# williamyang1991/VToonify

Measured on NVIDIA H100. Metric: frames/sec at 576x1024, higher is better.
Workload: dtype bf16x3 (fp32 operands split into bf16 hi+lo, 3 tensor-core products, fp32 accumulate)

## Files before the change

vtoonify_b200/_lib.py:

```python
import ctypes
import os
from ctypes import POINTER, Structure, c_char_p, c_float, c_int, c_int32, c_int64, c_void_p

_HERE = os.path.dirname(os.path.abspath(__file__))
LIB_PATH = os.path.join(_HERE, "lib", "libvtoonify_b200.so")
ABI_VERSION = 6
VT_MAX_TAPS = 36
ACT_NONE, ACT_LRELU, ACT_RELU_TANH = 0, 1, 2


class VtError(RuntimeError):
    pass


class ConvDesc(Structure):
    _fields_ = [
        ("struct_size", c_int32), ("n_src", c_int32),
        ("src", c_void_p * 2), ("src_c", c_int32 * 2), ("src_cstride", c_int32 * 2),
        ("B", c_int32), ("H", c_int32), ("W", c_int32), ("Ho", c_int32), ("Wo", c_int32),
        ("stride", c_int32), ("taps", c_int32),
        ("tap_dy", c_int32 * VT_MAX_TAPS), ("tap_dx", c_int32 * VT_MAX_TAPS), ("tap_w", c_int32 * VT_MAX_TAPS),
        ("tap_phase", c_int32 * VT_MAX_TAPS), ("n_phase", c_int32), ("out_cpitch", c_int32), ("phase_off", c_int64 * 4),
        ("weight", c_void_p), ("wB", c_int32), ("w_taps", c_int32), ("w_cstride", c_int32), ("Cout", c_int32),
        ("out", c_void_p), ("out_sb", c_int64), ("out_sy", c_int64), ("out_sx", c_int64),
# ... 83 lines not shown
    if _lib is not None:
        return _lib
    if not os.path.exists(LIB_PATH):
        raise VtError(
            f"{LIB_PATH} is missing: build it with `python -c 'import __graft_entry__ as g; g.build()'` "
            "(or vtoonify_b200/csrc/build.sh). vtoonify_b200 has no CPU / PyTorch fallback.")
    lib = ctypes.CDLL(LIB_PATH)
    for name, (res, args) in SYMBOLS.items():
        fn = getattr(lib, name)
        fn.restype = res
        fn.argtypes = args
    if lib.vt_abi_version() != ABI_VERSION:
        raise VtError(f"ABI mismatch: library reports {lib.vt_abi_version()}, binding expects {ABI_VERSION}")
    for env, key in (("VT_TC_MODE", b"tc_mode"), ("VT_TC_MT", b"tc_mt"), ("VT_TC_TGROUP", b"tc_tgroup"),
                     ("VT_TC_STAGE_POLICY", b"tc_stage_policy"), ("VT_TC_HALO_PCT", b"tc_halo_pct"), ("VT_TC_M_MAJOR", b"tc_m_major"),
                     ("VT_INSTNORM_CHUNKS", b"instnorm_chunks")):
        if os.environ.get(env) is not None and os.environ.get(env) != "":
            lib.vt_set_option(key, int(os.environ[env]))
    _lib = lib
    return lib


def check(status):
    if status != 0:
        raise VtError(load().vt_last_error().decode("utf-8", "replace"))


def launch_count():
    return int(load().vt_launch_count())
```

vtoonify_b200/csrc/conv_tc.cu:

```cuda
#include "tc_common.cuh"
#include <cuda_bf16.h>
#include <mutex>

using namespace vt_tc;

int vt_validate_conv_desc(const vt_conv_desc* d, const char* who);
extern int g_upfirdn_tiled;
extern int g_smalln_is;
extern int g_fir4;
extern int g_instnorm_chunks;

namespace {

constexpr int TILE_W = 8, TILE_H = 16, TILE_M = 128;
constexpr int KCH = 32;
constexpr int MAX_SMEM = 227 * 1024;
constexpr int MAX_BLOCK_N = 128;
constexpr int MAX_ACC_COLS = 128;
constexpr int STATS_WARPS = 8;

struct TcArgs {
  CUtensorMap in_map[2][4];
  CUtensorMap w_map;
  int n_src, kchunks[2], coff[2];
// ... 17 lines not shown
  int64_t out_sb, out_sy, out_sx, phase_off[4];
  int64_t pix_sb, pix_sy, pix_sx, phase_pix[4];
  int act, round_tf32;
  float slope, gain, alpha, beta;
  const float* rgb_w; const float* rgb_bias; const float* rgb_skip; const float* rgb_skip_kernel; float* rgb_out;
  const float* slope_vec;
  const float* src_scale[2];
  const float* src_affine[2];
  int src_cn[2];
  int64_t sc_sb, sc_sy, sc_sx;
  int in_w, in_h;
  int mma_n;
  int m_major;
  float* stats_ws;
  float acc_scale;
};

constexpr int TC_THREADS = 384;
constexpr int XFORM_WARPS = 3;
constexpr int CONSUMERS = 2;
constexpr int RELEASE_ARRIVALS = CONSUMERS * 4;

enum TcOp : int {
  OP_TF32 = 0,
  OP_BF16 = 1,
  OP_F16 = 2,
  OP_BF16_NSTACK = 3,
};

template <int NW, bool F16>
__device__ __forceinline__ void wgmma_split(float* acc, uint64_t a, uint64_t b, uint32_t accumulate) {
  if constexpr (NW == 32) {
    if constexpr (F16) wgmma_f16_n32(acc, a, b, accumulate); else wgmma_bf16_n32(acc, a, b, accumulate);
  } else if constexpr (NW == 64) {
    if constexpr (F16) wgmma_f16_n64(acc, a, b, accumulate); else wgmma_bf16_n64(acc, a, b, accumulate);
  } else {
// ... 12 lines not shown
      wgmma_tf32_n64(acc, adesc + 4, bdesc + 4, 1); wgmma_tf32_n64(acc, adesc + 6, bdesc + 6, 1);
    } else {
      wgmma_tf32_n128(acc, adesc, bdesc, first ^ 1u); wgmma_tf32_n128(acc, adesc + 2, bdesc + 2, 1);
      wgmma_tf32_n128(acc, adesc + 4, bdesc + 4, 1); wgmma_tf32_n128(acc, adesc + 6, bdesc + 6, 1);
    }
  } else {
    constexpr bool nstack = OP == OP_BF16_NSTACK;
    constexpr int ao[6] = {0, 2, 4, 6, 0, 2};
    constexpr int bo[6] = {0, 2, 0, 2, 4, 6};
#pragma unroll
    for (int i = 0; i < (nstack ? 4 : 6); ++i)
      wgmma_split<NW, OP == OP_F16>(acc, adesc + (uint64_t)ao[i], bdesc + (uint64_t)(nstack ? ao[i] : bo[i]), i == 0 ? (first ^ 1u) : 1u);
  }
}

template <int NW, int MT, int OP>
__global__ void __launch_bounds__(TC_THREADS, 1)
conv_tc_kernel(const __grid_constant__ TcArgs p) {
  static_assert(MT * NW <= MAX_ACC_COLS && (MT == 1 || MT == 2 || MT == 4), "accumulators of one work item exceed the register plan");
  static_assert(OP != OP_BF16_NSTACK || NW == 64, "the N-stacked form is the Cout == 32 layer at MMA N = 64");
  constexpr bool SPLIT = OP != OP_TF32;
  extern __shared__ uint8_t smem_raw[];
  const uint32_t smem_base = (smem_u32(smem_raw) + 1023u) & ~1023u;
  const uint32_t a_base = smem_base;
  const uint32_t b_base = a_base + (uint32_t)p.a_stages * p.a_stage_bytes;
  const uint32_t bar_base = b_base + (uint32_t)p.b_stages * p.b_stage_bytes;
  auto a_full = [&](int i) { return bar_base + 8u * i; };
  auto a_empty = [&](int i) { return bar_base + 64u + 8u * i; };
  auto b_full = [&](int i) { return bar_base + 128u + 8u * i; };
  auto b_empty = [&](int i) { return bar_base + 192u + 8u * i; };
  auto a_ready = [&](int i) { return bar_base + 256u + 8u * i; };

  const int warp = threadIdx.x >> 5, lane = threadIdx.x & 31;
  const int wg = threadIdx.x >> 7;

  if (warp == 0 && lane == 0) {
    for (int s = 0; s < p.n_src; ++s)
      for (int v = 0; v < 4; ++v) tma_prefetch_desc(&p.in_map[s][v]);
    tma_prefetch_desc(&p.w_map);
  }
  if (warp == 1 && lane == 0) {
    for (int i = 0; i < p.a_stages; ++i) { mbar_init(a_full(i), 1); mbar_init(a_empty(i), RELEASE_ARRIVALS); mbar_init(a_ready(i), XFORM_WARPS); }
    for (int i = 0; i < p.b_stages; ++i) { mbar_init(b_full(i), 1); mbar_init(b_empty(i), RELEASE_ARRIVALS); }
    fence_barrier_init();
    fence_proxy_async_smem();
  }
  __syncthreads();

  const int m_tiles = p.B * p.tiles_y * p.tiles_x;
  const int tiles_per_img = p.tiles_y * p.tiles_x;
  constexpr int item_w = TILE_W * MT;

  if (wg == 0) {
    if (warp == 0) {
      int a_st = 0, b_st = 0;
      uint32_t a_par = 0, b_par = 0;
      for (int tile = blockIdx.x; tile < p.total_tiles; tile += gridDim.x) {
        const int n_tile = p.m_major ? tile % p.n_tiles : tile / m_tiles, m = p.m_major ? tile / p.n_tiles : tile % m_tiles;
// ... 107 lines not shown
#pragma unroll
                for (int m4 = 0; m4 < 4; ++m4) {
                  asm volatile("st.shared.v4.b32 [%0], {%1, %2, %3, %4};" ::"r"(row + ((m4 ^ ph) << 4)), "r"(hi[4 * m4]), "r"(hi[4 * m4 + 1]), "r"(hi[4 * m4 + 2]), "r"(hi[4 * m4 + 3]) : "memory");
                  asm volatile("st.shared.v4.b32 [%0], {%1, %2, %3, %4};" ::"r"(row + (((m4 + 4) ^ ph) << 4)), "r"(lo[4 * m4]), "r"(lo[4 * m4 + 1]), "r"(lo[4 * m4 + 2]), "r"(lo[4 * m4 + 3]) : "memory");
                }
              }
              fence_proxy_async_smem();
              __syncwarp();
              if (lane == 0) mbar_arrive(a_ready(a_st));
              if (++a_st == p.a_stages) { a_st = 0; a_par ^= 1; }
            }
          }
        }
      }
    }
  } else {
    const int c = wg - 1;
    const int tw_ = (threadIdx.x & 127) >> 5;
    const bool leader = lane == 0;
    const int qd = lane & 3;
    float acc[MT][NW / 2];
#pragma unroll
    for (int g = 0; g < MT; ++g)
#pragma unroll
      for (int i = 0; i < NW / 2; ++i) acc[g][i] = 0.f;
    const float nw = (p.noise && p.noise_w) ? *p.noise_w : 0.f;
    int a_st = 0, b_st = 0;
    uint32_t a_par = 0, b_par = 0;
    const uint32_t tile_bytes_n = (uint32_t)p.mma_n * 128u;
    for (int tile = blockIdx.x; tile < p.total_tiles; tile += gridDim.x) {
      const int n_tile = p.m_major ? tile % p.n_tiles : tile / m_tiles, m = p.m_major ? tile / p.n_tiles : tile % m_tiles;
      const int b = m / tiles_per_img, rem = m % tiles_per_img;
      const int oy0 = (rem / p.tiles_x) * TILE_H, ox0 = (rem % p.tiles_x) * item_w;
      const int n0 = n_tile * p.block_n;
      uint32_t first = 1;
      int rel_a = -1, rel_b = -1;
      for (int s = 0; s < p.n_src; ++s) {
        for (int kc = 0; kc < p.kchunks[s]; ++kc) {
          if (p.halo) mbar_wait(SPLIT ? a_ready(a_st) : a_full(a_st), a_par);
          int gj = 0;
          for (int j = 0; j < p.n_steps; ++j) {
            if (!p.halo) mbar_wait(SPLIT ? a_ready(a_st) : a_full(a_st), a_par);
            if (gj == 0) mbar_wait(b_full(b_st), b_par);
            uint32_t a_addr = a_base + a_st * p.a_stage_bytes;
            uint32_t sbo = 1024;
            if (p.halo) {
              a_addr += (uint32_t)p.step_aoff[j];
              sbo = (uint32_t)p.step_sbo[j];
            }
            a_addr += 8u * (uint32_t)c * sbo;
            const uint64_t bdesc = make_smem_desc_sw128(b_base + b_st * p.b_stage_bytes + (uint32_t)gj * tile_bytes_n, 1024);
            const bool last_of_group = (gj == p.tgroup - 1);
            wgmma_fence();
#pragma unroll
            for (int g = 0; g < MT; ++g) {
              const uint64_t adesc = make_smem_desc_sw128(a_addr + (uint32_t)(g * TILE_W * 128), sbo);
              mma_step<NW, OP>(acc[g], adesc, bdesc, first);
            }
            wgmma_commit();
            wgmma_wait<1>();
            if (leader) {
              if (rel_a >= 0) mbar_arrive(a_empty(rel_a));
              if (rel_b >= 0) mbar_arrive(b_empty(rel_b));
            }
            rel_a = (!p.halo || j == p.n_steps - 1) ? a_st : -1;
            rel_b = last_of_group ? b_st : -1;
            first = 0;
            if (last_of_group) { gj = 0; if (++b_st == p.b_stages) { b_st = 0; b_par ^= 1; } } else { ++gj; }
            if (!p.halo || j == p.n_steps - 1) { if (++a_st == p.a_stages) { a_st = 0; a_par ^= 1; } }
          }
        }
      }
      wgmma_wait<0>();
#pragma unroll
      for (int g = 0; g < MT; ++g) wgmma_pin<NW / 2>(acc[g]);
      if (leader) {
        if (rel_a >= 0) mbar_arrive(a_empty(rel_a));
        if (rel_b >= 0) mbar_arrive(b_empty(rel_b));
      }

      const int r0 = 64 * c + 16 * tw_ + (lane >> 2);
      const int ty = r0 / TILE_W, tx = r0 % TILE_W;
      const int ph0 = n0 / p.Cout, nb0 = n0 - ph0 * p.Cout;
      const int nchunks = p.block_n / 32;
#pragma unroll
      for (int g = 0; g < MT; ++g) {
        int oy[2], ox[2];
        bool in_img[2];
        int64_t off0[2], pix0[2];
        float rgb[2][3] = {{0.f, 0.f, 0.f}, {0.f, 0.f, 0.f}};
#pragma unroll
        for (int h = 0; h < 2; ++h) {
          oy[h] = oy0 + ty + h; ox[h] = ox0 + g * TILE_W + tx;
          in_img[h] = oy[h] < p.Ho && ox[h] < p.Wo;
          off0[h] = (int64_t)b * p.out_sb + (int64_t)oy[h] * p.out_sy + (int64_t)ox[h] * p.out_sx;
          pix0[h] = (int64_t)b * p.pix_sb + (int64_t)oy[h] * p.pix_sy + (int64_t)ox[h] * p.pix_sx;
        }
        int ph = ph0, nb = nb0 - 32;
#pragma unroll
        for (int j = 0; j < NW / 32; ++j) {
          if (j >= nchunks) break;
          nb += 32;
          if (nb >= p.Cout) { nb -= p.Cout; ++ph; }
          float nz[2];
#pragma unroll
          for (int h = 0; h < 2; ++h) nz[h] = (p.noise && in_img[h]) ? nw * __ldg(p.noise + p.phase_pix[ph] + pix0[h]) : 0.f;
          float v[2][4][2];
#pragma unroll
          for (int k = 0; k < 4; ++k)
#pragma unroll
            for (int h = 0; h < 2; ++h)
#pragma unroll
              for (int e = 0; e < 2; ++e) {
                const int i = 16 * j + 4 * k + 2 * h + e;
                float x = acc[g][i];
                if constexpr (OP == OP_BF16_NSTACK) x += acc[g][(i + 16) % (NW / 2)];
                v[h][k][e] = x * p.acc_scale;
              }
#pragma unroll
          for (int k = 0; k < 4; ++k) {
            const int ch = nb + 8 * k + 2 * qd;
            float2 bq = make_float2(0.f, 0.f), sq = make_float2(p.slope, p.slope);
            if (p.bias) bq = __ldg(reinterpret_cast<const float2*>(p.bias + ch));
            if (p.slope_vec) sq = __ldg(reinterpret_cast<const float2*>(p.slope_vec + ch));
#pragma unroll
            for (int h = 0; h < 2; ++h) {
              float v0 = v[h][k][0] + bq.x + nz[h], v1 = v[h][k][1] + bq.y + nz[h];
              if (p.act == VT_ACT_LRELU) {
                v0 = vt_lrelu(v0, sq.x) * p.gain; v1 = vt_lrelu(v1, sq.y) * p.gain;
              } else if (p.act == VT_ACT_RELU_TANH) {
                v0 = tanhf(fmaxf(v0, 0.f)); v1 = tanhf(fmaxf(v1, 0.f));
              }
              const int64_t off = p.phase_off[ph] + off0[h] + ch;
              if (p.res) {
                if (in_img[h]) {
                  const float2 rv = __ldg(reinterpret_cast<const float2*>(p.res + off));
                  v0 = v0 * p.alpha + p.beta * rv.x; v1 = v1 * p.alpha + p.beta * rv.y;
                }
              } else if (p.alpha != 1.f) {
                v0 *= p.alpha; v1 *= p.alpha;
              }
              if (p.round_tf32) { v0 = vt_round_tf32(v0); v1 = vt_round_tf32(v1); }
              if (p.rgb_w) {
                const float* w0 = p.rgb_w + ((int64_t)(p.wB > 1 ? b : 0) * 3) * p.Cout + ch;
#pragma unroll
                for (int cc = 0; cc < 3; ++cc) {
                  const float2 wv = __ldg(reinterpret_cast<const float2*>(w0 + cc * p.Cout));
                  rgb[h][cc] = fmaf(v1, wv.y, fmaf(v0, wv.x, rgb[h][cc]));
                }
              }
              if (in_img[h] && p.out) *reinterpret_cast<float2*>(p.out + off) = make_float2(v0, v1);
              v[h][k][0] = in_img[h] ? v0 : 0.f; v[h][k][1] = in_img[h] ? v1 : 0.f;
            }
          }
          if (p.stats_ws) {
            const int kchunk = ((rem * MT + g) * STATS_WARPS) + c * 4 + tw_;
            float2* wsp = reinterpret_cast<float2*>(p.stats_ws) + ((int64_t)kchunk * p.B + b) * p.Cout + nb + 2 * qd;
#pragma unroll
            for (int k = 0; k < 4; ++k)
#pragma unroll
              for (int e = 0; e < 2; ++e) {
                float ssum = v[0][k][e] + v[1][k][e];
                float ssq = fmaf(v[0][k][e], v[0][k][e], v[1][k][e] * v[1][k][e]);
#pragma unroll
                for (int o = 4; o < 32; o <<= 1) {
                  ssum += __shfl_xor_sync(0xffffffffu, ssum, o);
                  ssq += __shfl_xor_sync(0xffffffffu, ssq, o);
                }
                if (lane < 4) wsp[8 * k + e] = make_float2(ssum, ssq);
              }
          }
        }
        if (p.rgb_w) {
#pragma unroll
          for (int h = 0; h < 2; ++h)
#pragma unroll
            for (int cc = 0; cc < 3; ++cc) {
              rgb[h][cc] += __shfl_xor_sync(0xffffffffu, rgb[h][cc], 1);
              rgb[h][cc] += __shfl_xor_sync(0xffffffffu, rgb[h][cc], 2);
            }
#pragma unroll
          for (int h = 0; h < 2; ++h) {
            if (qd != 0 || !in_img[h]) continue;
            const int py = oy[h], px = ox[h];
            float o[3] = {rgb[h][0] + __ldg(p.rgb_bias), rgb[h][1] + __ldg(p.rgb_bias + 1), rgb[h][2] + __ldg(p.rgb_bias + 2)};
            const int64_t HW = (int64_t)p.Ho * p.Wo;
            if (p.rgb_skip) {
              const int hs = p.Ho >> 1, ws = p.Wo >> 1;
              const int ky0 = (py - 2) & 1, kx0 = (px - 2) & 1;
              const int iy0 = (py - 2 + ky0) >> 1, ix0 = (px - 2 + kx0) >> 1;
              const float my0 = iy0 >= 0 ? 1.f : 0.f, my1 = (iy0 + 1) < hs ? 1.f : 0.f;
              const float mx0 = ix0 >= 0 ? 1.f : 0.f, mx1 = (ix0 + 1) < ws ? 1.f : 0.f;
              const int cy0 = iy0 < 0 ? 0 : iy0, cy1 = (iy0 + 1) < hs ? iy0 + 1 : hs - 1;
              const int cx0 = ix0 < 0 ? 0 : ix0, cx1 = (ix0 + 1) < ws ? ix0 + 1 : ws - 1;
              const float* kk = p.rgb_skip_kernel;
              const float w00 = __ldg(kk + (3 - ky0) * 4 + (3 - kx0)) * my0 * mx0;
              const float w01 = __ldg(kk + (3 - ky0) * 4 + (1 - kx0)) * my0 * mx1;
              const float w10 = __ldg(kk + (1 - ky0) * 4 + (3 - kx0)) * my1 * mx0;
              const float w11 = __ldg(kk + (1 - ky0) * 4 + (1 - kx0)) * my1 * mx1;
#pragma unroll
              for (int cc = 0; cc < 3; ++cc) {
                const float* sp = p.rgb_skip + ((int64_t)b * 3 + cc) * (int64_t)hs * ws;
                float u = __ldg(sp + (int64_t)cy0 * ws + cx0) * w00;
                u = fmaf(__ldg(sp + (int64_t)cy0 * ws + cx1), w01, u);
                u = fmaf(__ldg(sp + (int64_t)cy1 * ws + cx0), w10, u);
                u = fmaf(__ldg(sp + (int64_t)cy1 * ws + cx1), w11, u);
                o[cc] += u;
              }
            }
#pragma unroll
            for (int cc = 0; cc < 3; ++cc) p.rgb_out[((int64_t)b * 3 + cc) * HW + (int64_t)py * p.Wo + px] = o[cc];
          }
        }
      }
    }
  }
}

struct TcKernel {
  int nw, mt, op;
  void (*fn)(TcArgs);
};
#define VT_TC_OPS(NW, MT) {NW, MT, OP_TF32, conv_tc_kernel<NW, MT, OP_TF32>}, {NW, MT, OP_BF16, conv_tc_kernel<NW, MT, OP_BF16>}, \
                          {NW, MT, OP_F16, conv_tc_kernel<NW, MT, OP_F16>}
const TcKernel kTcKernels[] = {
    VT_TC_OPS(128, 1), VT_TC_OPS(64, 1), VT_TC_OPS(64, 2), VT_TC_OPS(32, 1), VT_TC_OPS(32, 2), VT_TC_OPS(32, 4),
    {64, 1, OP_BF16_NSTACK, conv_tc_kernel<64, 1, OP_BF16_NSTACK>}, {64, 2, OP_BF16_NSTACK, conv_tc_kernel<64, 2, OP_BF16_NSTACK>},
};
#undef VT_TC_OPS

}

typedef CUresult (*PFN_encodeTiled)(CUtensorMap*, CUtensorMapDataType, cuuint32_t, void*, const cuuint64_t*,
                                    const cuuint64_t*, const cuuint32_t*, const cuuint32_t*, CUtensorMapInterleave,
                                    CUtensorMapSwizzle, CUtensorMapL2promotion, CUtensorMapFloatOOBfill);

static PFN_encodeTiled get_encode() {
  static PFN_encodeTiled fn = nullptr;
  static std::once_flag once;
  std::call_once(once, [] {
    void* f = nullptr;
    cudaDriverEntryPointQueryResult qres;
    if (cudaGetDriverEntryPoint("cuTensorMapEncodeTiled", &f, cudaEnableDefault, &qres) == cudaSuccess &&
        qres == cudaDriverEntryPointSuccess)
// ... 21 lines not shown
}


namespace {
inline int make_map4(CUtensorMap* m, const void* base, const uint64_t dims[4], const uint64_t strides_b[3], const uint32_t box[4],
                     const char* what, bool bf16 = false) { return vt_tc_make_map4(m, base, dims, strides_b, box, what, bf16); }

int g_tc_mode = 1;
int g_tc_mt = 0;
int g_tc_transpose = 1;
int g_tc_tgroup = 0;
int g_tc_s2_halo = 0;
int g_tc_stage_policy = 1;
int g_tc_halo_pct = 60;
int g_tc_m_major = 1;

int check_supported(const vt_conv_desc* d, bool set_err) {
#define VT_SUP(cond, ...) do { if (!(cond)) { if (set_err) vt_set_error(__VA_ARGS__); return 0; } } while (0)
  VT_SUP(d->Cout % 32 == 0, "conv_tc: Cout must be a multiple of 32 (got %d)", d->Cout);
  VT_SUP(d->out != nullptr || d->rgb_w != nullptr, "conv_tc: out may be NULL only with the fused ToRGB tail (image-only launch)");
  for (int s = 0; s < d->n_src; ++s) {
    VT_SUP(d->src_c[s] % KCH == 0, "conv_tc: src_c[%d]=%d must be a multiple of 32", s, d->src_c[s]);
    VT_SUP(d->src_cstride[s] % 4 == 0, "conv_tc: channel stride must be a multiple of 4");
  }
  VT_SUP(d->stride == 1 || d->stride == 2, "conv_tc: stride must be 1 or 2");
  VT_SUP(d->n_phase == 1 || (d->n_phase == 4 && d->stride == 1 && g_tc_mode != 0 && !d->res), "conv_tc: phases need stride 1, halo mode, no residual");
  for (int ph = 0; ph < d->n_phase; ++ph) VT_SUP(d->phase_off[ph] % 4 == 0, "conv_tc: phase offset must be a multiple of 4 floats");
  VT_SUP(d->out_sx % 4 == 0 && d->out_sy % 4 == 0 && d->out_sb % 4 == 0, "conv_tc: output strides must be multiples of 4 floats");
  VT_SUP(((uintptr_t)d->out & 15) == 0, "conv_tc: out not 16-byte aligned");
  VT_SUP(d->w_cstride % 4 == 0, "conv_tc: weight stride must be a multiple of 4");
// ... 12 lines not shown
  return 1;
#undef VT_SUP
}

}

extern "C" int vt_set_option(const char* key, int value) {
  if (key && strcmp(key, "tc_mode") == 0) { int old = g_tc_mode; g_tc_mode = value; return old; }
  if (key && strcmp(key, "tc_mt") == 0) { int old = g_tc_mt; g_tc_mt = value; return old; }
  if (key && strcmp(key, "tc_tgroup") == 0) { int old = g_tc_tgroup; g_tc_tgroup = value; return old; }
  if (key && strcmp(key, "tc_s2_halo") == 0) { int old = g_tc_s2_halo; g_tc_s2_halo = value; return old; }
  if (key && strcmp(key, "tc_stage_policy") == 0) { int old = g_tc_stage_policy; g_tc_stage_policy = value; return old; }
  if (key && strcmp(key, "tc_halo_pct") == 0) { int old = g_tc_halo_pct; g_tc_halo_pct = value; return old; }
  if (key && strcmp(key, "tc_m_major") == 0) { int old = g_tc_m_major; g_tc_m_major = value; return old; }
  if (key && strcmp(key, "tc_transpose") == 0) { int old = g_tc_transpose; g_tc_transpose = value; return old; }
  if (key && strcmp(key, "instnorm_chunks") == 0) { int old = g_instnorm_chunks; g_instnorm_chunks = value; return old; }
  if (key && strcmp(key, "fir4") == 0) { int old = g_fir4; g_fir4 = value; return old; }
  if (key && strcmp(key, "smalln_is") == 0) { int old = g_smalln_is; g_smalln_is = value; return old; }
  if (key && strcmp(key, "upfirdn_tiled") == 0) { int old = g_upfirdn_tiled; g_upfirdn_tiled = value; return old; }
  return -1;
}

extern "C" int vt_conv2d_tc_supported(const vt_conv_desc* d) {
  if (!d || d->struct_size != (int)sizeof(vt_conv_desc)) return 0;
  return check_supported(d, false);
}

static int conv_tc_run(const vt_conv_desc* d, void* stream, int* chunks_out) {
  if (vt_validate_conv_desc(d, "conv2d_tc")) return 1;
  if (!check_supported(d, true)) return 1;
// ... 108 lines not shown
      halo_bytes = (int)(vt_cdiv(halo_bytes + w * h * 128, 1024) * 1024);
    }
    const int64_t tap_bytes = (int64_t)d->taps * TILE_M * 128;
    const bool pays = (d->stride == 2 && g_tc_s2_halo) ? (tx_bytes * 10 <= tap_bytes * 6) : ((int64_t)tx_bytes * 100 <= tap_bytes * g_tc_halo_pct);
    a.halo = can_halo && fits && halo_bytes <= 96 * 1024 && (mt > 1 || pays) &&
             2 * halo_bytes + 2 * bnm * 128 * tgroup + fixed <= MAX_SMEM;
    if (!a.halo && mt > 1) continue;
    a.halo_x0 = a.hv_x0[0]; a.halo_y0 = a.hv_y0[0]; a.halo_w = hv_w[a.hv_view[0]];
    a.a_tx_bytes = a.halo ? tx_bytes : TILE_M * 128;
    a.a_rows = a.halo ? (a.hv_off[a.n_hv - 1] + a.hv_bytes[a.n_hv - 1]) / 128 : TILE_M;
    a.a_stage_bytes = a.halo ? halo_bytes : TILE_M * 128;
    a.b_stage_bytes = bnm * 128 * tgroup;
    a.a_stages = a.halo ? 3 : 4;
    a.b_stages = tgroup > 1 ? 4 : 6;
    const int b_floor = (g_tc_stage_policy == 1 && a.halo && a.a_stage_bytes >= 40 * 1024 && tgroup == 1) ? 5 : 3;
    while (a.a_stages * a.a_stage_bytes + a.b_stages * a.b_stage_bytes + fixed > MAX_SMEM) {
      if (a.b_stages > b_floor) --a.b_stages;
      else if (a.a_stages > 2) --a.a_stages;
      else if (a.b_stages > 2) --a.b_stages;
      else break;
    }
    if (b_floor > 3)
      while (a.b_stages < 8 && a.a_stages * a.a_stage_bytes + (a.b_stages + 1) * a.b_stage_bytes + fixed <= MAX_SMEM) ++a.b_stages;
    smem_bytes = a.a_stages * a.a_stage_bytes + a.b_stages * a.b_stage_bytes + fixed;
    if (smem_bytes <= MAX_SMEM || mt == 1) break;
  }
  a.b_tx_bytes = bnm * 128 * tgroup;
  VT_CHECK(smem_bytes <= MAX_SMEM && a.a_stages >= 2 && a.b_stages >= 2 && a.a_stages <= 8 && a.b_stages <= 8,
           "conv_tc: shared memory plan does not fit (%d B, mt=%d, bn=%d)", smem_bytes, mt, bn);
  for (int t = 0; t < d->taps; ++t) {
    const int v = a.step_view[t];
    int i = 0;
    while (i < a.n_hv - 1 && a.hv_view[i] != v) ++i;
    a.step_aoff[t] = a.hv_off[i] + ((a.step_vy[t] - vy0[v]) * hv_w[v] + (a.step_vx[t] - vx0[v])) * 128;
    a.step_sbo[t] = (uint16_t)(hv_w[v] * 128);
  }
  a.block_n = bn;
  a.mma_n = bnm;
  a.n_tiles = n_eff / bn;
// ... 58 lines not shown
      if (make_map4(&a.w_map, d->weight_bf16x3, dims2, str2, box, "weight(bf16x3)", true)) return 1;
    } else {
      const uint32_t box[4] = {KCH, (uint32_t)bn, (uint32_t)a.tgroup, 1};
      if (make_map4(&a.w_map, d->weight, dims, str, box, "weight")) return 1;
    }
  }
  static std::once_flag attr_once;
  static cudaError_t attr_err = cudaSuccess;
  std::call_once(attr_once, [] {
    for (const TcKernel& k : kTcKernels)
      if (attr_err == cudaSuccess) attr_err = cudaFuncSetAttribute(k.fn, cudaFuncAttributeMaxDynamicSharedMemorySize, MAX_SMEM);
  });
  VT_CHECK(attr_err == cudaSuccess, "conv_tc: cudaFuncSetAttribute failed: %s", cudaGetErrorString(attr_err));
  const TcKernel* kern = nullptr;
  for (const TcKernel& k : kTcKernels)
    if (k.nw == bnm && k.mt == mt && k.op == op) kern = &k;
  if (!kern) return vt_set_error("conv_tc: no kernel for MMA N = %d, %d M tiles, operand mode %d", bnm, mt, op);
  int grid = vt_num_sms();
  if (grid > a.total_tiles) grid = a.total_tiles;
  kern->fn<<<grid, TC_THREADS, smem_bytes, (cudaStream_t)stream>>>(a);
  VT_LAUNCH_CHECK();
  return 0;
}

extern "C" int vt_conv2d_tc_tf32(const vt_conv_desc* d, void* stream) { return conv_tc_run(d, stream, nullptr); }

static bool rs_shape(const vt_conv_desc* d) {
  if (d->n_src != 1 || d->stride != 1 || d->taps != 9 || d->n_phase != 1 || d->res || d->slope_vec || !d->weight_bf16x3) return false;
  if (d->src_scale[0] || d->src_affine[0] || d->alpha != 1.f) return false;
  if ((d->Cout != 32 && d->Cout != 64) || (d->src_c[0] != 32 && d->src_c[0] != 64)) return false;
  return d->act == VT_ACT_NONE || d->act == VT_ACT_LRELU;
}

extern "C" int vt_conv2d_rs_supported(const vt_conv_desc* d) {
  if (!d || d->struct_size != (int)sizeof(vt_conv_desc)) return 0;
// ... 17 lines not shown
```

Baseline: 32.54.

## Add warp-specialized epilogue warpgroup with shared-memory accumulator slots

Adds a fourth warpgroup to the persistent tensor-core conv kernel. After the MMA mainloop, consumer warpgroups dump their accumulators into shared-memory slots guarded by mbarriers, and the new group runs the bias/activation/noise/residual/stats/ToRGB epilogue. This lets consumers start the next tile's MMAs while the epilogue runs. It is enabled by default for layers with large K and paid for with shared memory, which can shrink pipeline stages, plus extra smem traffic and 512-thread CTAs. Optional clock-based phase instrumentation is also added behind a compile flag.

```diff
diff --git a/vtoonify_b200/_lib.py b/vtoonify_b200/_lib.py
--- a/vtoonify_b200/_lib.py
+++ b/vtoonify_b200/_lib.py
@@ -121,6 +121,7 @@
         raise VtError(f"ABI mismatch: library reports {lib.vt_abi_version()}, binding expects {ABI_VERSION}")
     for env, key in (("VT_TC_MODE", b"tc_mode"), ("VT_TC_MT", b"tc_mt"), ("VT_TC_TGROUP", b"tc_tgroup"),
                      ("VT_TC_STAGE_POLICY", b"tc_stage_policy"), ("VT_TC_HALO_PCT", b"tc_halo_pct"), ("VT_TC_M_MAJOR", b"tc_m_major"),
+                     ("VT_TC_EPI_WS", b"tc_epi_ws"),
                      ("VT_INSTNORM_CHUNKS", b"instnorm_chunks")):
         if os.environ.get(env) is not None and os.environ.get(env) != "":
             lib.vt_set_option(key, int(os.environ[env]))
diff --git a/vtoonify_b200/csrc/conv_tc.cu b/vtoonify_b200/csrc/conv_tc.cu
--- a/vtoonify_b200/csrc/conv_tc.cu
+++ b/vtoonify_b200/csrc/conv_tc.cu
@@ -55,12 +55,43 @@
   int m_major;
   float* stats_ws;
   float acc_scale;
+  int acc_slots;
+  int slot_bytes;
 };
 
 constexpr int TC_THREADS = 384;
+constexpr int TC_THREADS_EPI = 512;
 constexpr int XFORM_WARPS = 3;
 constexpr int CONSUMERS = 2;
+constexpr int CONSUMER_THREADS = CONSUMERS * 128;
 constexpr int RELEASE_ARRIVALS = CONSUMERS * 4;
+
+enum TcPhase : int {
+  PH_ITEMS = 0, PH_CTA_NS, PH_CTA_CYC,
+  PH_WAIT_A, PH_WAIT_B, PH_MMA, PH_DRAIN,
+  PH_EPI, PH_SLOT_WAIT,
+  PH_EW_WAIT, PH_EW_WORK,
+  PH_COUNT
+};
+#ifdef VT_TC_PHASES
+__device__ unsigned long long g_tc_phase[PH_COUNT];
+struct PhaseClock {
+  unsigned long long acc[PH_COUNT];
+  long long t;
+  static __device__ __forceinline__ long long now() {
+    long long c;
+    asm volatile("mov.u64 %0, %%clock64;" : "=l"(c));
+    return c;
+  }
+  __device__ __forceinline__ PhaseClock() : acc{}, t(now()) {}
+  __device__ __forceinline__ void lap(int k) { const long long n = now(); acc[k] += (unsigned long long)(n - t); t = n; }
+  __device__ __forceinline__ void flush() { for (int k = 0; k < PH_COUNT; ++k) if (acc[k]) atomicAdd(&g_tc_phase[k], acc[k]); }
+};
+#else
+struct PhaseClock {
+  __device__ __forceinline__ void lap(int) {}
+};
+#endif
 
 enum TcOp : int {
   OP_TF32 = 0,
@@ -103,8 +134,150 @@
   }
 }
 
-template <int NW, int MT, int OP>
-__global__ void __launch_bounds__(TC_THREADS, 1)
+template <int NW, int MT, int OP, class Load4>
+__device__ __forceinline__ void tc_epilogue(const TcArgs& p, Load4 load4, int c, int tw_, int lane, int b, int rem, int oy0, int ox0,
+                                            int n0, float nw) {
+  const int qd = lane & 3;
+  const int r0 = 64 * c + 16 * tw_ + (lane >> 2);
+  const int ty = r0 / TILE_W, tx = r0 % TILE_W;
+  const int ph0 = n0 / p.Cout, nb0 = n0 - ph0 * p.Cout;
+  const int nchunks = p.block_n / 32;
+#pragma unroll
+  for (int g = 0; g < MT; ++g) {
+    int oy[2], ox[2];
+    bool in_img[2];
+    int64_t off0[2], pix0[2];
+    float rgb[2][3] = {{0.f, 0.f, 0.f}, {0.f, 0.f, 0.f}};
+#pragma unroll
+    for (int h = 0; h < 2; ++h) {
+      oy[h] = oy0 + ty + h; ox[h] = ox0 + g * TILE_W + tx;
+      in_img[h] = oy[h] < p.Ho && ox[h] < p.Wo;
+      off0[h] = (int64_t)b * p.out_sb + (int64_t)oy[h] * p.out_sy + (int64_t)ox[h] * p.out_sx;
+      pix0[h] = (int64_t)b * p.pix_sb + (int64_t)oy[h] * p.pix_sy + (int64_t)ox[h] * p.pix_sx;
+    }
+    int ph = ph0, nb = nb0 - 32;
+#pragma unroll
+    for (int j = 0; j < NW / 32; ++j) {
+      if (j >= nchunks) break;
+      nb += 32;
+      if (nb >= p.Cout) { nb -= p.Cout; ++ph; }
+      float nz[2];
+#pragma unroll
+      for (int h = 0; h < 2; ++h) nz[h] = (p.noise && in_img[h]) ? nw * __ldg(p.noise + p.phase_pix[ph] + pix0[h]) : 0.f;
+      float v[2][4][2];
+#pragma unroll
+      for (int k = 0; k < 4; ++k) {
+        const float4 q = load4(g, 16 * j + 4 * k);
+        float x[4] = {q.x, q.y, q.z, q.w};
+        if constexpr (OP == OP_BF16_NSTACK) {
+          const float4 q2 = load4(g, (16 * j + 4 * k + 16) % (NW / 2));
+          x[0] += q2.x; x[1] += q2.y; x[2] += q2.z; x[3] += q2.w;
+        }
+#pragma unroll
+        for (int h = 0; h < 2; ++h)
+#pragma unroll
+          for (int e = 0; e < 2; ++e) v[h][k][e] = x[2 * h + e] * p.acc_scale;
+      }
+#pragma unroll
+      for (int k = 0; k < 4; ++k) {
+        const int ch = nb + 8 * k + 2 * qd;
+        float2 bq = make_float2(0.f, 0.f), sq = make_float2(p.slope, p.slope);
+        if (p.bias) bq = __ldg(reinterpret_cast<const float2*>(p.bias + ch));
+        if (p.slope_vec) sq = __ldg(reinterpret_cast<const float2*>(p.slope_vec + ch));
+#pragma unroll
+        for (int h = 0; h < 2; ++h) {
+          float v0 = v[h][k][0] + bq.x + nz[h], v1 = v[h][k][1] + bq.y + nz[h];
+          if (p.act == VT_ACT_LRELU) {
+            v0 = vt_lrelu(v0, sq.x) * p.gain; v1 = vt_lrelu(v1, sq.y) * p.gain;
+          } else if (p.act == VT_ACT_RELU_TANH) {
+            v0 = tanhf(fmaxf(v0, 0.f)); v1 = tanhf(fmaxf(v1, 0.f));
+          }
+          const int64_t off = p.phase_off[ph] + off0[h] + ch;
+          if (p.res) {
+            if (in_img[h]) {
+              const float2 rv = __ldg(reinterpret_cast<const float2*>(p.res + off));
+              v0 = v0 * p.alpha + p.beta * rv.x; v1 = v1 * p.alpha + p.beta * rv.y;
+            }
+          } else if (p.alpha != 1.f) {
+            v0 *= p.alpha; v1 *= p.alpha;
+          }
+          if (p.round_tf32) { v0 = vt_round_tf32(v0); v1 = vt_round_tf32(v1); }
+          if (p.rgb_w) {
+            const float* w0 = p.rgb_w + ((int64_t)(p.wB > 1 ? b : 0) * 3) * p.Cout + ch;
+#pragma unroll
+            for (int cc = 0; cc < 3; ++cc) {
+              const float2 wv = __ldg(reinterpret_cast<const float2*>(w0 + cc * p.Cout));
+              rgb[h][cc] = fmaf(v1, wv.y, fmaf(v0, wv.x, rgb[h][cc]));
+            }
+          }
+          if (in_img[h] && p.out) *reinterpret_cast<float2*>(p.out + off) = make_float2(v0, v1);
+          v[h][k][0] = in_img[h] ? v0 : 0.f; v[h][k][1] = in_img[h] ? v1 : 0.f;
+        }
+      }
+      if (p.stats_ws) {
+        const int kchunk = ((rem * MT + g) * STATS_WARPS) + c * 4 + tw_;
+        float2* wsp = reinterpret_cast<float2*>(p.stats_ws) + ((int64_t)kchunk * p.B + b) * p.Cout + nb + 2 * qd;
+#pragma unroll
+        for (int k = 0; k < 4; ++k)
+#pragma unroll
+          for (int e = 0; e < 2; ++e) {
+            float ssum = v[0][k][e] + v[1][k][e];
+            float ssq = fmaf(v[0][k][e], v[0][k][e], v[1][k][e] * v[1][k][e]);
+#pragma unroll
+            for (int o = 4; o < 32; o <<= 1) {
+              ssum += __shfl_xor_sync(0xffffffffu, ssum, o);
+              ssq += __shfl_xor_sync(0xffffffffu, ssq, o);
+            }
+            if (lane < 4) wsp[8 * k + e] = make_float2(ssum, ssq);
+          }
+      }
+    }
+    if (p.rgb_w) {
+#pragma unroll
+      for (int h = 0; h < 2; ++h)
+#pragma unroll
+        for (int cc = 0; cc < 3; ++cc) {
+          rgb[h][cc] += __shfl_xor_sync(0xffffffffu, rgb[h][cc], 1);
+          rgb[h][cc] += __shfl_xor_sync(0xffffffffu, rgb[h][cc], 2);
+        }
+#pragma unroll
+      for (int h = 0; h < 2; ++h) {
+        if (qd != 0 || !in_img[h]) continue;
+        const int py = oy[h], px = ox[h];
+        float o[3] = {rgb[h][0] + __ldg(p.rgb_bias), rgb[h][1] + __ldg(p.rgb_bias + 1), rgb[h][2] + __ldg(p.rgb_bias + 2)};
+        const int64_t HW = (int64_t)p.Ho * p.Wo;
+        if (p.rgb_skip) {
+          const int hs = p.Ho >> 1, ws = p.Wo >> 1;
+          const int ky0 = (py - 2) & 1, kx0 = (px - 2) & 1;
+          const int iy0 = (py - 2 + ky0) >> 1, ix0 = (px - 2 + kx0) >> 1;
+          const float my0 = iy0 >= 0 ? 1.f : 0.f, my1 = (iy0 + 1) < hs ? 1.f : 0.f;
+          const float mx0 = ix0 >= 0 ? 1.f : 0.f, mx1 = (ix0 + 1) < ws ? 1.f : 0.f;
+          const int cy0 = iy0 < 0 ? 0 : iy0, cy1 = (iy0 + 1) < hs ? iy0 + 1 : hs - 1;
+          const int cx0 = ix0 < 0 ? 0 : ix0, cx1 = (ix0 + 1) < ws ? ix0 + 1 : ws - 1;
+          const float* kk = p.rgb_skip_kernel;
+          const float w00 = __ldg(kk + (3 - ky0) * 4 + (3 - kx0)) * my0 * mx0;
+          const float w01 = __ldg(kk + (3 - ky0) * 4 + (1 - kx0)) * my0 * mx1;
+          const float w10 = __ldg(kk + (1 - ky0) * 4 + (3 - kx0)) * my1 * mx0;
+          const float w11 = __ldg(kk + (1 - ky0) * 4 + (1 - kx0)) * my1 * mx1;
+#pragma unroll
+          for (int cc = 0; cc < 3; ++cc) {
+            const float* sp = p.rgb_skip + ((int64_t)b * 3 + cc) * (int64_t)hs * ws;
+            float u = __ldg(sp + (int64_t)cy0 * ws + cx0) * w00;
+            u = fmaf(__ldg(sp + (int64_t)cy0 * ws + cx1), w01, u);
+            u = fmaf(__ldg(sp + (int64_t)cy1 * ws + cx0), w10, u);
+            u = fmaf(__ldg(sp + (int64_t)cy1 * ws + cx1), w11, u);
+            o[cc] += u;
+          }
+        }
+#pragma unroll
+        for (int cc = 0; cc < 3; ++cc) p.rgb_out[((int64_t)b * 3 + cc) * HW + (int64_t)py * p.Wo + px] = o[cc];
+      }
+    }
+  }
+}
+
+template <int NW, int MT, int OP, bool EPI>
+__global__ void __launch_bounds__(EPI ? TC_THREADS_EPI : TC_THREADS, 1)
 conv_tc_kernel(const __grid_constant__ TcArgs p) {
   static_assert(MT * NW <= MAX_ACC_COLS && (MT == 1 || MT == 2 || MT == 4), "accumulators of one work item exceed the register plan");
   static_assert(OP != OP_BF16_NSTACK || NW == 64, "the N-stacked form is the Cout == 32 layer at MMA N = 64");
@@ -119,6 +292,9 @@
   auto b_full = [&](int i) { return bar_base + 128u + 8u * i; };
   auto b_empty = [&](int i) { return bar_base + 192u + 8u * i; };
   auto a_ready = [&](int i) { return bar_base + 256u + 8u * i; };
+  auto acc_full = [&](int i) { return bar_base + 320u + 8u * i; };
+  auto acc_empty = [&](int i) { return bar_base + 336u + 8u * i; };
+  auto slot_ptr = [&](int i) { return reinterpret_cast<float4*>(smem_raw + (bar_base + 1024u + (uint32_t)i * p.slot_bytes - smem_u32(smem_raw))); };
 
   const int warp = threadIdx.x >> 5, lane = threadIdx.x & 31;
   const int wg = threadIdx.x >> 7;
@@ -131,6 +307,8 @@
   if (warp == 1 && lane == 0) {
     for (int i = 0; i < p.a_stages; ++i) { mbar_init(a_full(i), 1); mbar_init(a_empty(i), RELEASE_ARRIVALS); mbar_init(a_ready(i), XFORM_WARPS); }
     for (int i = 0; i < p.b_stages; ++i) { mbar_init(b_full(i), 1); mbar_init(b_empty(i), RELEASE_ARRIVALS); }
+    if constexpr (EPI)
+      for (int i = 0; i < p.acc_slots; ++i) { mbar_init(acc_full(i), CONSUMER_THREADS); mbar_init(acc_empty(i), 128); }
     fence_barrier_init();
     fence_proxy_async_smem();
   }
@@ -268,11 +446,43 @@
         }
       }
     }
+  } else if (EPI && wg == 1 + CONSUMERS) {
+    PhaseClock pc;
+    const int t = threadIdx.x & 127;
+    const float nw = (p.noise && p.noise_w) ? *p.noise_w : 0.f;
+    int slot = 0;
+    uint32_t slot_par = 0;
+    for (int tile = blockIdx.x; tile < p.total_tiles; tile += gridDim.x) {
+      const int n_tile = p.m_major ? tile % p.n_tiles : tile / m_tiles, m = p.m_major ? tile / p.n_tiles : tile % m_tiles;
+      const int b = m / tiles_per_img, rem = m % tiles_per_img;
+      const int oy0 = (rem / p.tiles_x) * TILE_H, ox0 = (rem % p.tiles_x) * item_w;
+      mbar_wait(acc_full(slot), slot_par);
+      pc.lap(PH_EW_WAIT);
+      const float4* src = slot_ptr(slot);
+#pragma unroll 1
+      for (int c = 0; c < CONSUMERS; ++c) {
+        const float4* s = src + c * 128 + t;
+        tc_epilogue<NW, MT, OP>(p, [&](int g, int i) { return s[((g * NW / 2 + i) >> 2) * CONSUMER_THREADS]; }, c, t >> 5, lane, b, rem,
+                                oy0, ox0, n_tile * p.block_n, nw);
+      }
+      mbar_arrive(acc_empty(slot));
+      if (++slot == p.acc_slots) { slot = 0; slot_par ^= 1; }
+      pc.lap(PH_EW_WORK);
+    }
+#ifdef VT_TC_PHASES
+    if (t == 0) pc.flush();
+#endif
   } else {
+    PhaseClock pc;
+#ifdef VT_TC_PHASES
+    const uint64_t ns0 = globaltimer_ns();
+    const long long cyc0 = clock64();
+#endif
     const int c = wg - 1;
     const int tw_ = (threadIdx.x & 127) >> 5;
     const bool leader = lane == 0;
-    const int qd = lane & 3;
+    int slot = 0;
+    uint32_t slot_par = 0;
     float acc[MT][NW / 2];
 #pragma unroll
     for (int g = 0; g < MT; ++g)
@@ -291,11 +501,16 @@
       int rel_a = -1, rel_b = -1;
       for (int s = 0; s < p.n_src; ++s) {
         for (int kc = 0; kc < p.kchunks[s]; ++kc) {
+          pc.lap(PH_MMA);
           if (p.halo) mbar_wait(SPLIT ? a_ready(a_st) : a_full(a_st), a_par);
+          pc.lap(PH_WAIT_A);
           int gj = 0;
           for (int j = 0; j < p.n_steps; ++j) {
+            pc.lap(PH_MMA);
             if (!p.halo) mbar_wait(SPLIT ? a_ready(a_st) : a_full(a_st), a_par);
+            pc.lap(PH_WAIT_A);
             if (gj == 0) mbar_wait(b_full(b_st), b_par);
+            pc.lap(PH_WAIT_B);
             uint32_t a_addr = a_base + a_st * p.a_stage_bytes;
             uint32_t sbo = 1024;
             if (p.halo) {
@@ -325,6 +540,7 @@
           }
         }
       }
+      pc.lap(PH_MMA);
       wgmma_wait<0>();
 #pragma unroll
       for (int g = 0; g < MT; ++g) wgmma_pin<NW / 2>(acc[g]);
@@ -332,156 +548,63 @@
         if (rel_a >= 0) mbar_arrive(a_empty(rel_a));
         if (rel_b >= 0) mbar_arrive(b_empty(rel_b));
       }
-
-      const int r0 = 64 * c + 16 * tw_ + (lane >> 2);
-      const int ty = r0 / TILE_W, tx = r0 % TILE_W;
-      const int ph0 = n0 / p.Cout, nb0 = n0 - ph0 * p.Cout;
-      const int nchunks = p.block_n / 32;
-#pragma unroll
-      for (int g = 0; g < MT; ++g) {
-        int oy[2], ox[2];
-        bool in_img[2];
-        int64_t off0[2], pix0[2];
-        float rgb[2][3] = {{0.f, 0.f, 0.f}, {0.f, 0.f, 0.f}};
-#pragma unroll
-        for (int h = 0; h < 2; ++h) {
-          oy[h] = oy0 + ty + h; ox[h] = ox0 + g * TILE_W + tx;
-          in_img[h] = oy[h] < p.Ho && ox[h] < p.Wo;
-          off0[h] = (int64_t)b * p.out_sb + (int64_t)oy[h] * p.out_sy + (int64_t)ox[h] * p.out_sx;
-          pix0[h] = (int64_t)b * p.pix_sb + (int64_t)oy[h] * p.pix_sy + (int64_t)ox[h] * p.pix_sx;
-        }
-        int ph = ph0, nb = nb0 - 32;
-#pragma unroll
-        for (int j = 0; j < NW / 32; ++j) {
-          if (j >= nchunks) break;
-          nb += 32;
-          if (nb >= p.Cout) { nb -= p.Cout; ++ph; }
-          float nz[2];
-#pragma unroll
-          for (int h = 0; h < 2; ++h) nz[h] = (p.noise && in_img[h]) ? nw * __ldg(p.noise + p.phase_pix[ph] + pix0[h]) : 0.f;
-          float v[2][4][2];
-#pragma unroll
-          for (int k = 0; k < 4; ++k)
-#pragma unroll
-            for (int h = 0; h < 2; ++h)
-#pragma unroll
-              for (int e = 0; e < 2; ++e) {
-                const int i = 16 * j + 4 * k + 2 * h + e;
-                float x = acc[g][i];
-                if constexpr (OP == OP_BF16_NSTACK) x += acc[g][(i + 16) % (NW / 2)];
-                v[h][k][e] = x * p.acc_scale;
-              }
-#pragma unroll
-          for (int k = 0; k < 4; ++k) {
-            const int ch = nb + 8 * k + 2 * qd;
-            float2 bq = make_float2(0.f, 0.f), sq = make_float2(p.slope, p.slope);
-            if (p.bias) bq = __ldg(reinterpret_cast<const float2*>(p.bias + ch));
-            if (p.slope_vec) sq = __ldg(reinterpret_cast<const float2*>(p.slope_vec + ch));
-#pragma unroll
-            for (int h = 0; h < 2; ++h) {
-              float v0 = v[h][k][0] + bq.x + nz[h], v1 = v[h][k][1] + bq.y + nz[h];
-              if (p.act == VT_ACT_LRELU) {
-                v0 = vt_lrelu(v0, sq.x) * p.gain; v1 = vt_lrelu(v1, sq.y) * p.gain;
-              } else if (p.act == VT_ACT_RELU_TANH) {
-                v0 = tanhf(fmaxf(v0, 0.f)); v1 = tanhf(fmaxf(v1, 0.f));
-              }
-              const int64_t off = p.phase_off[ph] + off0[h] + ch;
-              if (p.res) {
-                if (in_img[h]) {
-                  const float2 rv = __ldg(reinterpret_cast<const float2*>(p.res + off));
-                  v0 = v0 * p.alpha + p.beta * rv.x; v1 = v1 * p.alpha + p.beta * rv.y;
-                }
-              } else if (p.alpha != 1.f) {
-                v0 *= p.alpha; v1 *= p.alpha;
-              }
-              if (p.round_tf32) { v0 = vt_round_tf32(v0); v1 = vt_round_tf32(v1); }
-              if (p.rgb_w) {
-                const float* w0 = p.rgb_w + ((int64_t)(p.wB > 1 ? b : 0) * 3) * p.Cout + ch;
-#pragma unroll
-                for (int cc = 0; cc < 3; ++cc) {
-                  const float2 wv = __ldg(reinterpret_cast<const float2*>(w0 + cc * p.Cout));
-                  rgb[h][cc] = fmaf(v1, wv.y, fmaf(v0, wv.x, rgb[h][cc]));
-                }
-              }
-              if (in_img[h] && p.out) *reinterpret_cast<float2*>(p.out + off) = make_float2(v0, v1);
-              v[h][k][0] = in_img[h] ? v0 : 0.f; v[h][k][1] = in_img[h] ? v1 : 0.f;
-            }
-          }
-          if (p.stats_ws) {
-            const int kchunk = ((rem * MT + g) * STATS_WARPS) + c * 4 + tw_;
-            float2* wsp = reinterpret_cast<float2*>(p.stats_ws) + ((int64_t)kchunk * p.B + b) * p.Cout + nb + 2 * qd;
-#pragma unroll
-            for (int k = 0; k < 4; ++k)
-#pragma unroll
-              for (int e = 0; e < 2; ++e) {
-                float ssum = v[0][k][e] + v[1][k][e];
-                float ssq = fmaf(v[0][k][e], v[0][k][e], v[1][k][e] * v[1][k][e]);
-#pragma unroll
-                for (int o = 4; o < 32; o <<= 1) {
-                  ssum += __shfl_xor_sync(0xffffffffu, ssum, o);
-                  ssq += __shfl_xor_sync(0xffffffffu, ssq, o);
-                }
-                if (lane < 4) wsp[8 * k + e] = make_float2(ssum, ssq);
-              }
-          }
-        }
-        if (p.rgb_w) {
-#pragma unroll
-          for (int h = 0; h < 2; ++h)
-#pragma unroll
-            for (int cc = 0; cc < 3; ++cc) {
-              rgb[h][cc] += __shfl_xor_sync(0xffffffffu, rgb[h][cc], 1);
-              rgb[h][cc] += __shfl_xor_sync(0xffffffffu, rgb[h][cc], 2);
-            }
-#pragma unroll
-          for (int h = 0; h < 2; ++h) {
-            if (qd != 0 || !in_img[h]) continue;
-            const int py = oy[h], px = ox[h];
-            float o[3] = {rgb[h][0] + __ldg(p.rgb_bias), rgb[h][1] + __ldg(p.rgb_bias + 1), rgb[h][2] + __ldg(p.rgb_bias + 2)};
-            const int64_t HW = (int64_t)p.Ho * p.Wo;
-            if (p.rgb_skip) {
-              const int hs = p.Ho >> 1, ws = p.Wo >> 1;
-              const int ky0 = (py - 2) & 1, kx0 = (px - 2) & 1;
-              const int iy0 = (py - 2 + ky0) >> 1, ix0 = (px - 2 + kx0) >> 1;
-              const float my0 = iy0 >= 0 ? 1.f : 0.f, my1 = (iy0 + 1) < hs ? 1.f : 0.f;
-              const float mx0 = ix0 >= 0 ? 1.f : 0.f, mx1 = (ix0 + 1) < ws ? 1.f : 0.f;
-              const int cy0 = iy0 < 0 ? 0 : iy0, cy1 = (iy0 + 1) < hs ? iy0 + 1 : hs - 1;
-              const int cx0 = ix0 < 0 ? 0 : ix0, cx1 = (ix0 + 1) < ws ? ix0 + 1 : ws - 1;
-              const float* kk = p.rgb_skip_kernel;
-              const float w00 = __ldg(kk + (3 - ky0) * 4 + (3 - kx0)) * my0 * mx0;
-              const float w01 = __ldg(kk + (3 - ky0) * 4 + (1 - kx0)) * my0 * mx1;
-              const float w10 = __ldg(kk + (1 - ky0) * 4 + (3 - kx0)) * my1 * mx0;
-              const float w11 = __ldg(kk + (1 - ky0) * 4 + (1 - kx0)) * my1 * mx1;
-#pragma unroll
-              for (int cc = 0; cc < 3; ++cc) {
-                const float* sp = p.rgb_skip + ((int64_t)b * 3 + cc) * (int64_t)hs * ws;
-                float u = __ldg(sp + (int64_t)cy0 * ws + cx0) * w00;
-                u = fmaf(__ldg(sp + (int64_t)cy0 * ws + cx1), w01, u);
-                u = fmaf(__ldg(sp + (int64_t)cy1 * ws + cx0), w10, u);
-                u = fmaf(__ldg(sp + (int64_t)cy1 * ws + cx1), w11, u);
-                o[cc] += u;
-              }
-            }
-#pragma unroll
-            for (int cc = 0; cc < 3; ++cc) p.rgb_out[((int64_t)b * 3 + cc) * HW + (int64_t)py * p.Wo + px] = o[cc];
-          }
-        }
-      }
-    }
+      pc.lap(PH_DRAIN);
+      if constexpr (EPI) {
+        mbar_wait(acc_empty(slot), slot_par ^ 1);
+        pc.lap(PH_SLOT_WAIT);
+        float4* dst = slot_ptr(slot) + c * 128 + (threadIdx.x & 127);
+#pragma unroll
+        for (int g = 0; g < MT; ++g)
+#pragma unroll
+          for (int q = 0; q < NW / 8; ++q)
+            dst[(g * NW / 8 + q) * CONSUMER_THREADS] = make_float4(acc[g][4 * q], acc[g][4 * q + 1], acc[g][4 * q + 2], acc[g][4 * q + 3]);
+        mbar_arrive(acc_full(slot));
+        if (++slot == p.acc_slots) { slot = 0; slot_par ^= 1; }
+      } else {
+        tc_epilogue<NW, MT, OP>(p, [&](int g, int i) { return make_float4(acc[g][i], acc[g][i + 1], acc[g][i + 2], acc[g][i + 3]); }, c,
+                                tw_, lane, b, rem, oy0, ox0, n0, nw);
+      }
+      pc.lap(PH_EPI);
+#ifdef VT_TC_PHASES
+      pc.acc[PH_ITEMS] += 1;
+#endif
+    }
+#ifdef VT_TC_PHASES
+    if (threadIdx.x == 128) {
+      pc.acc[PH_CTA_NS] = globaltimer_ns() - ns0;
+      pc.acc[PH_CTA_CYC] = (unsigned long long)(clock64() - cyc0);
+      pc.flush();
+    }
+#endif
   }
 }
 
 struct TcKernel {
-  int nw, mt, op;
+  int nw, mt, op, epi;
   void (*fn)(TcArgs);
 };
-#define VT_TC_OPS(NW, MT) {NW, MT, OP_TF32, conv_tc_kernel<NW, MT, OP_TF32>}, {NW, MT, OP_BF16, conv_tc_kernel<NW, MT, OP_BF16>}, \
-                          {NW, MT, OP_F16, conv_tc_kernel<NW, MT, OP_F16>}
+#define VT_TC_K(NW, MT, OP) {NW, MT, OP, 0, conv_tc_kernel<NW, MT, OP, false>}, {NW, MT, OP, 1, conv_tc_kernel<NW, MT, OP, true>}
+#define VT_TC_OPS(NW, MT) VT_TC_K(NW, MT, OP_TF32), VT_TC_K(NW, MT, OP_BF16), VT_TC_K(NW, MT, OP_F16)
 const TcKernel kTcKernels[] = {
     VT_TC_OPS(128, 1), VT_TC_OPS(64, 1), VT_TC_OPS(64, 2), VT_TC_OPS(32, 1), VT_TC_OPS(32, 2), VT_TC_OPS(32, 4),
-    {64, 1, OP_BF16_NSTACK, conv_tc_kernel<64, 1, OP_BF16_NSTACK>}, {64, 2, OP_BF16_NSTACK, conv_tc_kernel<64, 2, OP_BF16_NSTACK>},
+    VT_TC_K(64, 1, OP_BF16_NSTACK), VT_TC_K(64, 2, OP_BF16_NSTACK),
 };
 #undef VT_TC_OPS
+#undef VT_TC_K
+
+}
+
+#ifdef VT_TC_PHASES
+extern "C" int vt_tc_phase_read(unsigned long long* out) {
+  static const unsigned long long zero[PH_COUNT] = {};
+  VT_CHECK(cudaDeviceSynchronize() == cudaSuccess && cudaMemcpyFromSymbol(out, g_tc_phase, sizeof(zero)) == cudaSuccess &&
+               cudaMemcpyToSymbol(g_tc_phase, zero, sizeof(zero)) == cudaSuccess,
+           "vt_tc_phase_read: copy failed");
+  return 0;
+}
+#endif
+
+namespace {
 
 }
 
@@ -533,6 +656,8 @@
 int g_tc_stage_policy = 1;
 int g_tc_halo_pct = 60;
 int g_tc_m_major = 1;
+int g_tc_epi_ws = 1;
+constexpr int EPI_WS_MIN_K = 1024;
 
 int check_supported(const vt_conv_desc* d, bool set_err) {
 #define VT_SUP(cond, ...) do { if (!(cond)) { if (set_err) vt_set_error(__VA_ARGS__); return 0; } } while (0)
@@ -575,6 +700,7 @@
   if (key && strcmp(key, "tc_halo_pct") == 0) { int old = g_tc_halo_pct; g_tc_halo_pct = value; return old; }
   if (key && strcmp(key, "tc_m_major") == 0) { int old = g_tc_m_major; g_tc_m_major = value; return old; }
   if (key && strcmp(key, "tc_transpose") == 0) { int old = g_tc_transpose; g_tc_transpose = value; return old; }
+  if (key && strcmp(key, "tc_epi_ws") == 0) { int old = g_tc_epi_ws; g_tc_epi_ws = value; return old; }
   if (key && strcmp(key, "instnorm_chunks") == 0) { int old = g_instnorm_chunks; g_instnorm_chunks = value; return old; }
   if (key && strcmp(key, "fir4") == 0) { int old = g_fir4; g_fir4 = value; return old; }
   if (key && strcmp(key, "smalln_is") == 0) { int old = g_smalln_is; g_smalln_is = value; return old; }
@@ -713,15 +839,25 @@
     a.a_stages = a.halo ? 3 : 4;
     a.b_stages = tgroup > 1 ? 4 : 6;
     const int b_floor = (g_tc_stage_policy == 1 && a.halo && a.a_stage_bytes >= 40 * 1024 && tgroup == 1) ? 5 : 3;
-    while (a.a_stages * a.a_stage_bytes + a.b_stages * a.b_stage_bytes + fixed > MAX_SMEM) {
-      if (a.b_stages > b_floor) --a.b_stages;
-      else if (a.a_stages > 2) --a.a_stages;
-      else if (a.b_stages > 2) --a.b_stages;
-      else break;
+    a.slot_bytes = mt * bnm * CONSUMER_THREADS * 2;
+    const int ring_bytes = a.a_stages * a.a_stage_bytes + a.b_stages * a.b_stage_bytes + fixed;
+    const bool epi_ws = g_tc_epi_ws == 2 || (g_tc_epi_ws == 1 && (coff * d->taps) >= EPI_WS_MIN_K);
+    a.acc_slots = !epi_ws ? 0 : ring_bytes + 2 * a.slot_bytes <= MAX_SMEM ? 2 : 1;
+    for (;;) {
+      const int a0 = a.a_stages, b0 = a.b_stages;
+      while (a.a_stages * a.a_stage_bytes + a.b_stages * a.b_stage_bytes + a.acc_slots * a.slot_bytes + fixed > MAX_SMEM) {
+        if (a.b_stages > b_floor) --a.b_stages;
+        else if (a.a_stages > 2) --a.a_stages;
+        else if (a.b_stages > 2) --a.b_stages;
+        else break;
+      }
+      if (a.acc_slots == 0 || a.a_stages * a.a_stage_bytes + a.b_stages * a.b_stage_bytes + a.acc_slots * a.slot_bytes + fixed <= MAX_SMEM) break;
+      a.acc_slots = 0; a.a_stages = a0; a.b_stages = b0;
     }
     if (b_floor > 3)
-      while (a.b_stages < 8 && a.a_stages * a.a_stage_bytes + (a.b_stages + 1) * a.b_stage_bytes + fixed <= MAX_SMEM) ++a.b_stages;
-    smem_bytes = a.a_stages * a.a_stage_bytes + a.b_stages * a.b_stage_bytes + fixed;
+      while (a.b_stages < 8 && a.a_stages * a.a_stage_bytes + (a.b_stages + 1) * a.b_stage_bytes + a.acc_slots * a.slot_bytes + fixed <= MAX_SMEM)
+        ++a.b_stages;
+    smem_bytes = a.a_stages * a.a_stage_bytes + a.b_stages * a.b_stage_bytes + a.acc_slots * a.slot_bytes + fixed;
     if (smem_bytes <= MAX_SMEM || mt == 1) break;
   }
   a.b_tx_bytes = bnm * 128 * tgroup;
@@ -810,11 +946,11 @@
   VT_CHECK(attr_err == cudaSuccess, "conv_tc: cudaFuncSetAttribute failed: %s", cudaGetErrorString(attr_err));
   const TcKernel* kern = nullptr;
   for (const TcKernel& k : kTcKernels)
-    if (k.nw == bnm && k.mt == mt && k.op == op) kern = &k;
+    if (k.nw == bnm && k.mt == mt && k.op == op && k.epi == (a.acc_slots > 0)) kern = &k;
   if (!kern) return vt_set_error("conv_tc: no kernel for MMA N = %d, %d M tiles, operand mode %d", bnm, mt, op);
   int grid = vt_num_sms();
   if (grid > a.total_tiles) grid = a.total_tiles;
-  kern->fn<<<grid, TC_THREADS, smem_bytes, (cudaStream_t)stream>>>(a);
+  kern->fn<<<grid, kern->epi ? TC_THREADS_EPI : TC_THREADS, smem_bytes, (cudaStream_t)stream>>>(a);
   VT_LAUNCH_CHECK();
   return 0;
 }
```

New measurement: 33.31, median of 6. 1.02x the previous value.
